# andrew-sha/CUDAFluidSimulator

Measured on AMD Instinct MI355X. Metric: particle-steps/sec (first 41 of the 100 steps of -m time), higher is better.
Workload: dtype f32

## Files before the change

cudafluidsimulator_amd/csrc/sph_api.hip:

```cpp
#include "sph_c_api.h"
#include "sph_device.h"

#include <hsa/hsa.h>
#include <hsa/hsa_ext_amd.h>

#include <algorithm>
#include <chrono>
#include <cmath>
#include <cstdio>
#include <cstdlib>
#include <cstring>
#include <string>
#include <vector>

namespace {

thread_local std::string g_create_error;

constexpr int kEventRing = 64;
constexpr int kCounterWords = 16 + 256 * 16;
constexpr size_t kCursorBytes = (size_t)SL_POOL_SHARDS * SL_CURSOR_STRIDE * sizeof(unsigned long long);

struct PairEvent {
    hipEvent_t a = nullptr, b = nullptr;
// ... 10 lines not shown

}

struct sph_handle {
    SphSettings settings{};
    SphOptions opt{};
    DevParams P{};
    int n = 0, cap = 0, device = 0;
    hipStream_t compute = nullptr, copy = nullptr;
    float4 *pos4[2] = {nullptr, nullptr};
    float4 *vel4[2] = {nullptr, nullptr};
    int cur = 0;
    int sorted = -1;
    SortWorkspace ws{};
    int sortedKeyBuf = 0;
    int2 *cellRange = nullptr;
    int2 *cellTable[2] = {nullptr, nullptr};
    int cellCur = 0;
    bool gridAhead = false;
    int2 *clickTable = nullptr;
    bool clickValid = false;
    bool aheadEnabled = true;
    StepEvents *aheadEv = nullptr;
    float *devPos[2] = {nullptr, nullptr};
    float *hostPos = nullptr;
    bool hostPosIsInit = false;
    float4 *stage[2] = {nullptr, nullptr};
    hipEvent_t stageFree[2] = {nullptr, nullptr};
    bool mappedPos = false;
    hipGraphExec_t stepGraph[2][3] = {{nullptr, nullptr, nullptr}, {nullptr, nullptr, nullptr}};
    StepEvents graphEv[2];
    bool graphEvPending[2] = {false, false};
    bool useGraph = false, capturing = false;
    int graphKeyBuf = 0;
    int graphCellCur[2] = {0, 0};
    hipEvent_t computeDone[2] = {nullptr, nullptr}, copyDone[2] = {nullptr, nullptr};
    bool copyPending[2] = {false, false};
    bool sdmaOk = false, stepTimed = false;
    hsa_agent_t hsaGpu{}, hsaCpu{};
    hsa_signal_t rbSig[2]{};
    bool rbPending[2] = {false, false};
    int rbDeferredSlot = -1;
    uint32_t sdmaEngine = 0;
    double hsaTickSeconds = 0;
    bool cursorClean = false;
    long long stepIndex = 0;
    float4 *force4 = nullptr;
    unsigned long long *pairCounter = nullptr;
    unsigned long long *pairHost = nullptr;
    StepEvents ring[kEventRing];
    int ringHead = 0;
    StepEvents *curEv = nullptr;
    SphKernelTimes kt{};
    float4 *pv8 = nullptr;
    uint32_t *maskPool = nullptr, *maskOff = nullptr;
    uint32_t *noneList = nullptr;
    uint32_t *hitCount = nullptr;
    int slabOwnedBegin = 0, slabOwnedEnd = 0;
    uint32_t *quiet = nullptr;
    float4 *quietVref = nullptr;
    unsigned long long *calm = nullptr;
    float4 *initPos4 = nullptr;
    SphOobLog *oobHost = nullptr;
    uint32_t oobSeen = 0;
    bool trace = false;
    double trEnqueue = 0, trSync = 0, trPost = 0, trBetween = 0, trPh[5] = {0, 0, 0, 0, 0};
    long long trSteps = 0;
    std::chrono::steady_clock::time_point trLastReturn{};
    hipEvent_t trBase = nullptr;
    int initZLayers = 0;
    bool useQuiet = true;
    uint64_t hitsRecorded = 0;
    unsigned long long *maskCursor = nullptr;
    unsigned long long maskCapacity = 0;
    bool external = false;
    hipStream_t ownCompute = nullptr;
    int *boundsDev = nullptr, *boundsHost = nullptr;
    int *partTiles = nullptr;
    PairEvent pairs[kPairRing];
    int pairHead = 0;
    int zLayers = 0;
    int tileChunkEnv = -1;
    int tileRotate = -1;
    RenderParams rp{};
    uint32_t *rDepth = nullptr, *rCount = nullptr, *rEdge = nullptr, *rRgb = nullptr;
    uint8_t *frameHost = nullptr;
    hipEvent_t frameDrawn = nullptr, frameCopied = nullptr;
    bool framePending = false;
    bool frameValid = false;
    double renderSeconds = 0;
    long long renderFrames = 0;
    bool ready = false;
    bool gridValid = false;
    int phase = 0;
    std::string err;
};

namespace {

#define HIPCHK(h, call)                                                               \
    do {                                                                              \
        hipError_t e__ = (call);                                                      \
        if (e__ != hipSuccess) {                                                      \
            (h)->err = std::string(#call) + ": " + hipGetErrorString(e__);            \
            return SPH_EHIP;                                                          \
        }                                                                             \
    } while (0)

#define SPH_ON_DEVICE(h)                                                              \
    do {                                                                              \
        int d__ = -1;                                                                 \
        if (hipGetDevice(&d__) != hipSuccess || d__ != (h)->device)                    \
            HIPCHK(h, hipSetDevice((h)->device));                                     \
    } while (0)

void report_oob(sph_handle *h) {
    if (!h || !h->oobHost) return;
    const uint32_t cnt = h->oobHost->count;
    if (cnt == h->oobSeen) return;
    const int D = h->P.D;
    const uint32_t shown = cnt < SPH_OOB_RECORDS ? cnt : SPH_OOB_RECORDS;
    for (uint32_t k = h->oobSeen < shown ? h->oobSeen : shown; k < shown; ++k) {
        const auto &r = h->oobHost->rec[k];
        const char axis[3] = {'x', 'y', 'z'};
        for (int a = 0; a < 3; ++a)
            if (r.cell[a] < 0 || r.cell[a] >= D)
                printf("OOB particle: %c = %d\n(%f, %f, %f)\n", axis[a], r.cell[a], r.pos[0], r.pos[1], r.pos[2]);
    }
    if (cnt > shown) printf("OOB particle: %u positions outside the grid so far (the first %u listed)\n", cnt, shown);
    fflush(stdout);
    h->oobSeen = cnt;
}

int fail(sph_handle *h, int code, const std::string &msg) {
    if (h) h->err = msg;
    else g_create_error = msg;
    return code;
}

float force_cut2(float h) {
    float h2 = h * h;
    float x = h2;
    for (int k = 0; k < 64; ++k) {
        float nx = std::nextafterf(x, INFINITY);
        if (sqrtf(nx) <= h) x = nx;
        else break;
    }
    return x;
}

void fill_params(sph_handle *h) {
    const SphSettings &s = h->settings;
    DevParams &P = h->P;
    P.h = s.h;
    P.h2 = s.h * s.h;
    P.vcoef = s.v_kernel_coeff;
    P.dcoef = s.d_kernel_coeff;
    P.boxDim = s.boxDim;
    P.boxHi = s.boxDim - s.h;
    P.dt = s.timestep;
    P.cut2 = force_cut2(s.h);
    P.D = (int)s.numCellsPerDim;
    P.morton = h->opt.key_order == SPH_KEY_MORTON ? 1 : 0;
    {
        SphSettings ref{};
        sph_default_settings(&ref, s.numParticles, s.randomInit);
// ... 401 lines not shown
    SPH_ON_DEVICE(h);
    if (h->external) return fail(h, SPH_ESTATE, "handle is in slab mode (external state)");
    if (n != h->n) return fail(h, SPH_EINVAL, "particle count differs from settings");
    const float hh = h->settings.h;
    const int D = h->P.D;
    std::vector<float4> p4((size_t)n), v4((size_t)n);
    int zmin = D, zmax = -1;
    for (int i = 0; i < n; ++i) {
        float x = pos[3 * i], y = pos[3 * i + 1], z = pos[3 * i + 2];
        const float qx = x / hh, qy = y / hh, qz = z / hh, Df = (float)D;
        if (!(qx >= 0.f && qx < Df && qy >= 0.f && qy < Df && qz >= 0.f && qz < Df && x >= 0.f && y >= 0.f && z >= 0.f))
            return fail(h, SPH_EINVAL, "position outside the simulation box");
        const int cz = (int)qz;
        zmin = cz < zmin ? cz : zmin;
        zmax = cz > zmax ? cz : zmax;
        uint32_t id = (uint32_t)i;
        float idbits;
        memcpy(&idbits, &id, 4);
        p4[i] = make_float4(x, y, z, idbits);
        v4[i] = vel ? make_float4(vel[3 * i], vel[3 * i + 1], vel[3 * i + 2], 0.f)
                    : make_float4(0.f, 0.f, 0.f, 0.f);
    }
    HIPCHK(h, hipStreamSynchronize(h->compute));
    HIPCHK(h, hipStreamSynchronize(h->copy));
    h->cur = 0;
    if (n > 0) {
        int rc = staged_upload(h, h->pos4[0], (size_t)n,
                               [&](size_t k, float4 *dst, size_t cnt) { memcpy(dst, p4.data() + k, cnt * sizeof(float4)); });
        if (!rc)
            rc = staged_upload(h, h->vel4[0], (size_t)n,
                               [&](size_t k, float4 *dst, size_t cnt) { memcpy(dst, v4.data() + k, cnt * sizeof(float4)); });
        if (rc) return rc;
    }
    HIPCHK(h, hipDeviceSynchronize());
    h->zLayers = zmax >= zmin ? zmax - zmin + 1 : 0;
    state_replaced(h);
    h->hostPosIsInit = false;
    if (h->hostPos && n > 0) memcpy(h->hostPos, pos, (size_t)n * 3 * sizeof(float));
    return SPH_OK;
}

static int slab_rotate(const sph_handle *h) { return h->tileRotate >= 0 ? h->tileRotate : 1; }

int tile_chunk(const sph_handle *h, int count, int layers) {
    if (h->tileChunkEnv >= 0) return h->tileChunkEnv;
    if (layers <= 0) return 0;
    const long long tiles = ((long long)count + 255) / 256;
    return (int)(tiles / (8ll * layers));
}

SweepArgs make_sweep_args(sph_handle *h) {
    SweepArgs A{};
    const int s = h->sorted;
    A.pos4 = h->pos4[s];
    A.vel4 = h->vel4[s];
    A.cellRange = h->cellRange;
    A.keys = h->ws.keys[h->sortedKeyBuf];
    A.pos_out = h->pos4[s ^ 1];
    A.vel_out = h->vel4[s ^ 1];
    A.host_order_pos = nullptr;
    A.force_out = h->force4;
    A.pairCounter = nullptr;
    A.i_begin = 0;
    A.i_end = h->n;
    A.i_origin = 0;
    A.i_begin2 = A.i_end2 = 0;
    A.nblk1 = 0;
    A.patchHalo = 0;
    A.n_all = h->n;
    A.tileChunk = tile_chunk(h, h->n, h->zLayers);
    A.tileRotate = h->tileRotate > 0 ? h->tileRotate : 0;
    A.maskPool = h->maskPool;
    A.maskOff = h->maskOff;
    A.noneList = h->noneList;
    A.hitCount = h->hitCount;
    A.maskCursor = h->maskCursor;
    A.maskCapacity = h->maskCapacity;
    A.pv8 = h->pv8;
    A.quiet = (h->useQuiet && h->quiet) ? h->quiet : nullptr;
    A.calm = h->calm;
    A.quietAll = A.quiet ? reinterpret_cast<uint32_t *>(h->quietVref + 1) : nullptr;
    A.quietHalo = nullptr;
    A.rhoToVel4 = h->external ? 1 : 0;
    A.listHead = reinterpret_cast<const int *>(h->cellRange);
    A.listNext = reinterpret_cast<const int *>(h->ws.vals[0]);
    return A;
}

GatherExtras gather_extras(sph_handle *h) {
    GatherExtras X;
    if (h->maskCursor) {
        X.cursor = h->maskCursor;
        X.cursorWords = (int)(kCursorBytes / sizeof(unsigned long long));
        h->cursorClean = true;
    }
    if (h->quiet && h->useQuiet) {
        X.vref = h->quietVref;
        X.calm = h->calm;
        X.quietAll = reinterpret_cast<uint32_t *>(h->quietVref + 1);
        if (h->external) {
            X.quietClear = h->quiet;
            X.quietWords = (int)(2 * (((size_t)h->cap + 63) / 64) + 2);
        }
    }
    return X;
}

int begin_step_events(sph_handle *h) {
    StepEvents &se = h->ring[h->ringHead];
    if (se.used) {
        int rc = resolve_events(h, se);
        if (rc) return rc;
    }
    se.used = true;
    se.counted = false;
    se.hasCopy = false;
    h->curEv = &se;
    h->ringHead = (h->ringHead + 1) % kEventRing;
    return SPH_OK;
}

int resolve_pair(sph_handle *h, PairEvent &pe) {
    if (!pe.used) return SPH_OK;
    float ms = 0.f;
    HIPCHK(h, hipEventSynchronize(pe.b));
    HIPCHK(h, hipEventElapsedTime(&ms, pe.a, pe.b));
    *pe.target += ms * 1e-3;
    pe.used = false;
    return SPH_OK;
}

int pair_begin(sph_handle *h, double *target, PairEvent **out, hipStream_t stream = nullptr) {
    PairEvent &pe = h->pairs[h->pairHead];
    int rc = resolve_pair(h, pe);
    if (rc) return rc;
    h->pairHead = (h->pairHead + 1) % kPairRing;
    pe.target = target;
    pe.used = true;
    HIPCHK(h, hipEventRecord(pe.a, stream ? stream : h->compute));
    *out = &pe;
    return SPH_OK;
}

int slab_range_ok(sph_handle *h, int buf, int i_begin, int i_end, int n_all) {
    if (!h->external || !h->pos4[0]) return fail(h, SPH_ESTATE, "sph_bind_buffers first");
    if ((buf != 0 && buf != 1) || i_begin < 0 || i_end < i_begin || n_all < i_end || n_all > h->cap)
        return fail(h, SPH_EINVAL, "bad slab range");
    return SPH_OK;
}

}

extern "C" {

int sph_set_stream(sph_handle *h, void *hip_stream) {
    if (!h) return SPH_EINVAL;
    SPH_ON_DEVICE(h);
    HIPCHK(h, hipStreamSynchronize(h->compute));
    if (!h->ownCompute) h->ownCompute = h->compute;
    h->compute = (hipStream_t)hip_stream;
    return SPH_OK;
}

int sph_bind_buffers(sph_handle *h, void *pos4_a, void *vel4_a, void *pos4_b, void *vel4_b,
                     int capacity) {
    if (!h) return SPH_EINVAL;
// ... 272 lines not shown
    float h = .1f;
    float h_pow_6 = (float)pow((double)h, 6.0);
    float h_pow_9 = (float)pow((double)h, 9.0);
    float v_kernel_coeff = 45.f / (3.14159265f * h_pow_6);
    float d_kernel_coeff = 315.f / (64.f * 3.14159265f * h_pow_9);
    memset(out, 0, sizeof(*out));
    out->randomInit = randomInit ? 1 : 0;
    out->numParticles = numParticles;
    out->h = h;
    out->v_kernel_coeff = v_kernel_coeff;
    out->d_kernel_coeff = d_kernel_coeff;
    out->boxDim = 10.f;
    out->numCellsPerDim = 100;
    out->timestep = (float).01;
    return SPH_OK;
}

int sph_initial_positions(const SphSettings *settings, float *pos_xyz) {
    if (!settings || (!pos_xyz && settings->numParticles > 0) || settings->numParticles < 0)
        return SPH_EINVAL;
    int written = init_positions_reference(*settings, pos_xyz);
    if (written < settings->numParticles) {
        fprintf(stderr,
                "sph: -i grid holds at most %d lattice points in the reference "
                "(simulator.cu:439-452); n=%d uses the dense-lattice EXTENSION\n",
                written, settings->numParticles);
        init_positions_dense(*settings, pos_xyz);
    }
    return SPH_OK;
}

int sph_create(const SphSettings *settings, const SphOptions *options, sph_handle **out) {
    if (!settings || !out) return fail(nullptr, SPH_EINVAL, "null argument");
    *out = nullptr;
    if (settings->numParticles < 0) return fail(nullptr, SPH_EINVAL, "numParticles < 0");
    if (!(settings->h > 0.f) || !(settings->numCellsPerDim >= 1.f) ||
        settings->numCellsPerDim > 1024.f)
        return fail(nullptr, SPH_EINVAL, "bad h / numCellsPerDim");
    int count = 0;
    if (hipGetDeviceCount(&count) != hipSuccess || count <= 0)
        return fail(nullptr, SPH_ENODEV,
                    "no HIP device: libsph_hip has no CPU fallback by design");
    sph_handle *h = new (std::nothrow) sph_handle();
    if (!h) return fail(nullptr, SPH_ENOMEM, "out of host memory");
    h->settings = *settings;
    if (options) {
        size_t sz = options->struct_size > 0 ? (size_t)options->struct_size : sizeof(SphOptions);
        memcpy(&h->opt, options, sz < sizeof(SphOptions) ? sz : sizeof(SphOptions));
    } else {
        h->opt.device = -1;
    }
    h->opt.struct_size = (int32_t)sizeof(SphOptions);
    if (h->opt.math_mode != SPH_MATH_STRICT && h->opt.math_mode != SPH_MATH_FAST) {
        delete h;
        return fail(nullptr, SPH_EINVAL, "unknown math_mode");
    }
    if (h->opt.sweep < SPH_SWEEP_LIST || h->opt.sweep > SPH_SWEEP_LINKED) {
        delete h;
        return fail(nullptr, SPH_EINVAL, "unknown sweep variant");
    }
    if (h->opt.math_mode == SPH_MATH_FAST &&
        (h->opt.sweep == SPH_SWEEP_DIRECT || h->opt.sweep == SPH_SWEEP_LINKED)) {
        delete h;
        return fail(nullptr, SPH_EINVAL, "SPH_MATH_FAST does not exist for SPH_SWEEP_DIRECT/LINKED");
    }
    if (h->opt.key_order != SPH_KEY_FLATTENED && h->opt.key_order != SPH_KEY_MORTON) {
        delete h;
        return fail(nullptr, SPH_EINVAL, "unknown key_order");
    }
    if (h->opt.key_order == SPH_KEY_MORTON &&
        (h->opt.sweep != SPH_SWEEP_DIRECT || (h->opt.flags & SPH_FLAG_EXTERNAL_STATE))) {
        delete h;
        return fail(nullptr, SPH_EINVAL, "SPH_KEY_MORTON is served by SPH_SWEEP_DIRECT, single domain, only");
    }
    if (h->opt.sweep == SPH_SWEEP_LINKED && (h->opt.flags & SPH_FLAG_EXTERNAL_STATE)) {
        delete h;
        return fail(nullptr, SPH_EINVAL, "SPH_SWEEP_LINKED is single-domain only");
    }
    h->n = settings->numParticles;
    if ((h->opt.flags & SPH_FLAG_EXTERNAL_STATE) && h->opt.capacity > 0) h->cap = h->opt.capacity;
    else h->cap = h->opt.capacity > h->n ? h->opt.capacity : h->n;
    if (const char *e = getenv("SPH_TILE_CHUNK")) h->tileChunkEnv = atoi(e);
    if (const char *e = getenv("SPH_XCD_ROTATE")) h->tileRotate = atoi(e);
    if (const char *e = getenv("SPH_STEP_TRACE")) h->trace = atoi(e) != 0;
    fill_params(h);
    int rc = SPH_OK;
    do {
        if (h->opt.device >= 0) {
            if (h->opt.device >= count) { rc = fail(nullptr, SPH_EINVAL, "device ordinal out of range"); break; }
            if (hipSetDevice(h->opt.device) != hipSuccess) { rc = fail(nullptr, SPH_EHIP, "hipSetDevice failed"); break; }
        }
        if (hipGetDevice(&h->device) != hipSuccess) { rc = fail(nullptr, SPH_EHIP, "hipGetDevice failed"); break; }
        if (hipStreamCreateWithFlags(&h->compute, hipStreamNonBlocking) != hipSuccess ||
            hipStreamCreateWithFlags(&h->copy, hipStreamNonBlocking) != hipSuccess) {
            rc = fail(nullptr, SPH_EHIP, "hipStreamCreate failed");
            break;
        }
        rc = alloc_device(h);
        if (rc) g_create_error = h->err;
    } while (0);
    if (rc) {
        sph_destroy(h);
        return rc;
    }
    *out = h;
    return SPH_OK;
}

void sph_destroy(sph_handle *h) {
    if (!h) return;
    if (h->trace && h->trSteps > 0)
        fprintf(stderr, "sph step trace (host, us per timed step over %lld steps): enqueue %.1f | wait for the compute stream %.1f | "
                        "after the wait %.1f | caller between two steps %.1f\n", h->trSteps, h->trEnqueue / h->trSteps * 1e6,
                h->trSync / h->trSteps * 1e6, h->trPost / h->trSteps * 1e6, h->trBetween / (h->trSteps > 1 ? h->trSteps - 1 : 1) * 1e6),
        fprintf(stderr, "  enqueue split: events %.1f | grid %.1f | density %.1f | force %.1f | read-back %.1f\n", h->trPh[0] / h->trSteps * 1e6,
                h->trPh[1] / h->trSteps * 1e6, h->trPh[2] / h->trSteps * 1e6, h->trPh[3] / h->trSteps * 1e6, h->trPh[4] / h->trSteps * 1e6);
    if (h->compute) (void)hipStreamSynchronize(h->compute);
    if (h->copy) (void)hipStreamSynchronize(h->copy);
    if (h->hsaTickSeconds > 0) {
        (void)sdma_wait(h, 0);
        (void)sdma_wait(h, 1);
        (void)hsa_signal_destroy(h->rbSig[0]);
        (void)hsa_signal_destroy(h->rbSig[1]);
        (void)hsa_shut_down();
    }
    for (int b = 0; b < 2; ++b) {
        if (h->pos4[b] && !h->external) (void)hipFree(h->pos4[b]);
        if (h->vel4[b] && !h->external) (void)hipFree(h->vel4[b]);
        if (h->ws.keys[b]) (void)hipFree(h->ws.keys[b]);
        if (h->ws.vals[b]) (void)hipFree(h->ws.vals[b]);
        if (h->devPos[b] && !h->mappedPos) (void)hipFree(h->devPos[b]);
        if (h->computeDone[b]) (void)hipEventDestroy(h->computeDone[b]);
        if (h->copyDone[b]) (void)hipEventDestroy(h->copyDone[b]);
    }
    if (h->ws.blockHist) (void)hipFree(h->ws.blockHist);
    if (h->ws.digitTotal) (void)hipFree(h->ws.digitTotal);
    for (auto &t : h->cellTable) if (t) (void)hipFree(t);
    if (h->hostPos) (void)hipHostFree(h->hostPos);
    for (int b = 0; b < 2; ++b) {
        if (h->stage[b]) (void)hipHostFree(h->stage[b]);
        if (h->stageFree[b]) (void)hipEventDestroy(h->stageFree[b]);
    }
    if (h->force4) (void)hipFree(h->force4);
    if (h->pairCounter) (void)hipFree(h->pairCounter);
    if (h->pairHost) (void)hipHostFree(h->pairHost);
    for (auto &se : h->ring) {
        for (auto &e : se.e) if (e) (void)hipEventDestroy(e);
        for (auto &e : se.c) if (e) (void)hipEventDestroy(e);
    }
    for (auto &se : h->graphEv) {
        for (auto &e : se.e) if (e) (void)hipEventDestroy(e);
        for (auto &e : se.c) if (e) (void)hipEventDestroy(e);
    }
    for (auto &gs : h->stepGraph)
        for (auto &g : gs)
            if (g) (void)hipGraphExecDestroy(g);
    if (h->pv8) (void)hipFree(h->pv8);
    if (h->maskPool) (void)hipFree(h->maskPool);
    if (h->maskOff) (void)hipFree(h->maskOff);
    if (h->noneList) (void)hipFree(h->noneList);
    if (h->hitCount) (void)hipFree(h->hitCount);
    if (h->maskCursor) (void)hipFree(h->maskCursor);
    if (h->quiet) (void)hipFree(h->quiet);
    if (h->quietVref) (void)hipFree(h->quietVref);
    if (h->calm) (void)hipFree(h->calm);
    if (h->initPos4) (void)hipFree(h->initPos4);
// ... 822 lines not shown
```

cudafluidsimulator_amd/csrc/sph_device.h:

```cpp
#pragma once

#include <hip/hip_runtime.h>
#include <stdint.h>

#define SPH_WAVE 64

#define SPH_MASS 0.02f
#define SPH_GAS_CONSTANT 1.f
#define SPH_REST_DENSITY 1000.f
#define SPH_VISCOSITY 1.f
#define SPH_GRAVITY -9.8f
#define SPH_ELASTICITY 0.5f
#define SPH_EPS_F (1e-4f)
#define SPH_PUSH_STRENGTH (5.f)
#define SPH_BOX_MAX_X (600)
#define SPH_BOX_MIN_X (200)
#define SPH_BOX_MAX_Y (450)
#define SPH_BOX_MIN_Y (150)

struct DevParams {
    float h;
    float h2;
    float vcoef;
    float dcoef;
// ... 38 lines not shown
    const float4 *velSample;
    float4 *vrefOut;
};
size_t sph_sort_workspace_blocks(int n);
int sph_sort_pairs(const SortWorkspace &ws, int n, int bits, hipStream_t s);
struct DevParams;
int sph_sort_cells(const SortWorkspace &ws, const DevParams &P, const float4 *pos4, int n, int bits,
                   hipStream_t s, int2 *cellRange, int numCells);

void sph_launch_hash(const DevParams &P, const float4 *pos4, uint32_t *keys,
                     uint32_t *vals, int n, hipStream_t s);
struct Thresholds { uint32_t v[8]; };
struct GatherExtras {
    unsigned long long *cursor = nullptr;
    int cursorWords = 0;
    int *bounds = nullptr;
    const float4 *vref = nullptr;
    unsigned long long *calm = nullptr;
    uint32_t *quietAll = nullptr;
    uint32_t *quietClear = nullptr;
    int quietWords = 0;
    Thresholds thr{};
    int nthr = 0;
};
void sph_launch_gather(const float4 *pos_in, const float4 *vel_in,
                       const uint32_t *perm, const uint32_t *sorted_keys,
                       float4 *pos_out, float4 *vel_out, float4 *pv8, int2 *cellRange, int n,
                       hipStream_t s, const GatherExtras &X = GatherExtras());
void sph_launch_lower_bounds(const uint32_t *sorted_keys, int n, Thresholds thr, int nthr,
                             int *bounds_dev, hipStream_t s);
void sph_launch_classify(const DevParams &P, const float4 *pos4, Thresholds thr, int nthr,
                         uint32_t *keys, uint32_t *vals, int n, hipStream_t s);
void sph_launch_partition(const DevParams &P, const float4 *pos_in, const float4 *vel_in, float4 *pos_out,
                          float4 *vel_out, Thresholds thr, int nthr, int n, int *tileCount, int *bounds_dev,
                          hipStream_t s);
size_t sph_partition_tiles(int n);
void sph_launch_gather_plain(const float4 *pos_in, const float4 *vel_in, const uint32_t *perm,
                             float4 *pos_out, float4 *vel_out, int n, hipStream_t s);
struct SegmentTable {
    const float4 *spos[8];
    const float4 *svel[8];
    int dst[8];
    int prefix[9];
    int n;
};
void sph_launch_copy_segments(const SegmentTable &T, float4 *dpos, float4 *dvel, hipStream_t s);
void sph_launch_click(const DevParams &P, const int2 *cellRange, float4 *vel4,
                      int mx, int my, hipStream_t s, int zlo = 0, int zhi = 1 << 30);

#define SL_POOL_SHARDS 64
#define SL_CURSOR_STRIDE 32

struct SweepArgs {
    const float4 *pos4;
    float4 *vel4;
    const int2 *cellRange;
    const uint32_t *keys;
    float4 *pos_out;
    float4 *vel_out;
    float *host_order_pos;
    float4 *force_out;
    unsigned long long *pairCounter;
    unsigned long long *stampCounter;
    int i_begin, i_end;
    int i_origin;
    int i_begin2, i_end2;
    int nblk1;
    int n_all;
    int patchHalo;
    int tileChunk;
    int tileRotate;
    uint32_t *maskPool;
    uint32_t *maskOff;
    uint32_t *hitCount;
    unsigned long long *maskCursor;
    uint32_t *noneList;
    unsigned long long maskCapacity;
    float4 *pv8;
    uint32_t *quiet;
    const unsigned long long *calm;
    uint32_t *quietAll;
    const uint32_t *quietHalo;
    int rhoToVel4;
    const int *listHead;
    const int *listNext;
};
void sph_launch_halo_quiet(const float4 *pv8, int lo_end, int hi_begin, int n_all, const float4 *vref,
                           const uint32_t *ownedQuiet, uint32_t *haloQuiet, hipStream_t s);
void sph_launch_link_build(const DevParams &P, const float4 *pos4, int *head, int *next, int n,
                           hipStream_t s);
void sph_launch_density_linked(const DevParams &P, const SweepArgs &A, hipStream_t s);
void sph_launch_force_linked(const DevParams &P, const SweepArgs &A, hipStream_t s);
void sph_launch_density_list(const DevParams &P, const SweepArgs &A, int mathMode, hipStream_t s);
void sph_launch_force_list(const DevParams &P, const SweepArgs &A, int mathMode, hipStream_t s);
void sph_launch_patch_halo(const SweepArgs &A, hipStream_t s);
void sph_launch_density(const DevParams &P, const SweepArgs &A, int mathMode,
                        int sweep, hipStream_t s);
void sph_launch_force(const DevParams &P, const SweepArgs &A, int mathMode,
                      int sweep, hipStream_t s);

struct RenderParams {
    int width, height;
    float Wf, Hf;
    int radius;
    int shade;
};
void sph_launch_render_edges(const RenderParams &R, uint32_t *edge, hipStream_t s);
void sph_launch_render(const RenderParams &R, const float4 *pos4, int n, bool plain, uint32_t *depth, uint32_t *count,
                       const uint32_t *edge, uint32_t *rgb, hipStream_t s);
```

cudafluidsimulator_amd/csrc/sweeps_list.hip:

```cpp
#include "sweep_common.h"

#define SL_NONE 0xFFFFFFFFu

#ifndef SL_WINDOW
#define SL_WINDOW 160
#endif
#ifndef SL_K1_THREADS
#define SL_K1_THREADS 64
#endif

#ifndef SL_K1_WAVES
#define SL_K1_WAVES 6
#endif
__device__ __forceinline__ void sl_store_quiet(const SweepArgs &A, int i, bool valid, float rho, int lane) {
    const unsigned long long calm = A.calm[(i - lane) >> 6];
    const float prs = fmaxf(0.f, SPH_GAS_CONSTANT * (rho - SPH_REST_DENSITY));
    const bool q = valid && prs == 0.f && ((calm >> lane) & 1ull);
    const unsigned long long qb = __ballot(q), vb = __ballot(valid);
    if (lane == 0) {
        reinterpret_cast<unsigned long long *>(A.quiet)[(i - lane) >> 6] = qb;
        if (A.quietAll && qb != vb) *A.quietAll = 0u;
    }
}
__device__ __forceinline__ uint32_t sl_quiet_window(const uint32_t *__restrict__ quiet, uint32_t j) {
// ... 131 lines not shown
                const int jsr = R.jsr, len = R.len;
                const float4 *cur = stage + (jsr - R.u0);
                const float4 *gcur = A.pos4 + jsr;
                uint32_t m = 0;
                int k = 0;
                auto trip = [&](const float4 (&pj)[SW_UNROLL]) {
#pragma unroll
                    for (int u = 0; u < SW_UNROLL; ++u) {
                        float dx = pi.x - pj[u].x;
                        float dy = pi.y - pj[u].y;
                        float dz = pi.z - pj[u].z;
                        float dist2;
                        float draw;
                        if (FAST) {
                            dist2 = __builtin_fmaf(dz, dz, __builtin_fmaf(dy, dy, dx * dx));
                            draw = h2v - dist2;
                            const float diff = fmaxf(draw, 0.f);
                            rho = __builtin_fmaf((massv * dcv) * (diff * diff), diff, rho);
                        } else {
                            dist2 = dx * dx + dy * dy + dz * dz;
                            draw = h2v - dist2;
                            float diff;
                            asm("v_max_f32_e32 %0, 0, %1" : "=v"(diff) : "v"(draw));
                            rho += massv * (dcv * diff * diff * diff);
                        }
                        if (SAMECUT) {
                            m = __builtin_amdgcn_alignbit(m, __float_as_uint(draw), 31);
                            continue;
                        }
                        asm("v_cmp_ngt_f32_e32 vcc, %1, %2\n\tv_addc_co_u32_e32 %0, vcc, %0, %0, vcc"
                            : "+v"(m)
                            : "v"(dist2), "v"(cut2r)
                            : "vcc");
                    }
#pragma unroll
                    for (int u = 0; u < SW_UNROLL; ++u) asm volatile("" ::"v"(pj[u].w));
                    if (((k + SW_UNROLL) & 31) == 0) {
                        if (SAMECUT) emit((uint32_t)(jsr + (k & ~31)), ~__builtin_bitreverse32(m));
                        else emit((uint32_t)(jsr + (k & ~31)), __builtin_bitreverse32(m));
                        m = 0;
                    }
                };
                if (R.staged) {
                    for (; __ballot(k < len); k += SW_UNROLL) {
                        float4 pj[SW_UNROLL];
#pragma unroll
                        for (int u = 0; u < SW_UNROLL; ++u) {
                            const float4 *p = (k + u < len) ? cur + k : sent;
                            pj[u] = p[u];
                        }
                        trip(pj);
                    }
                } else {
                    for (; __ballot(k < len); k += SW_UNROLL) {
                        float4 pj[SW_UNROLL];
#pragma unroll
                        for (int u = 0; u < SW_UNROLL; ++u) {
                            const bool in = k + u < len;
                            pj[u] = gcur[in ? k + u : 0];
                            pj[u].x = in ? pj[u].x : 1e18f;
                        }
                        trip(pj);
                    }
                }
                if ((k & 31) != 0) {
                    if (SAMECUT) emit((uint32_t)(jsr + (k & ~31)), (~__builtin_bitreverse32(m)) >> (32 - (k & 31)));
                    else emit((uint32_t)(jsr + (k & ~31)), __builtin_bitreverse32(m) >> (32 - (k & 31)));
                }
                __builtin_amdgcn_fence(__ATOMIC_ACQUIRE, "wavefront");
                __builtin_amdgcn_wave_barrier();
            }
        }
    }
    if (ok && valid) {
        if (pending) myq[(size_t)qidx * SPH_WAVE] = make_uint4(pj0, pm0, 0u, 0u);
        else if (qidx < Q) myq[(size_t)qidx * SPH_WAVE] = make_uint4(0u, 0u, 0u, 0u);
    }
    if (valid) {
        rho = fmaxf(rho, SPH_EPS_F);
        if (A.rhoToVel4) A.vel4[i].w = rho;
        A.pv8[2 * (size_t)i + 1].w = rho;
    }
    if (A.quiet) sl_store_quiet(A, i, valid, rho, lane);
    if (A.hitCount && valid) A.hitCount[i] = hcount;
}

#ifndef SL_SORT_SHIFT
#define SL_SORT_SHIFT 3
#endif
#define SL_DEAL_THREADS 256
#define SL_DEAL_ROWS SL_DEAL_THREADS
#define SL_DEAL_WINDOW (SL_DEAL_ROWS + SL_WINDOW - SPH_WAVE)
static_assert(SL_WINDOW >= SPH_WAVE, "the dealt sweep needs the window");

template <bool FAST, bool SLIM>
__global__ __launch_bounds__(SL_DEAL_THREADS) void k_force_dealt(DevParams P, SweepArgs A) {
    __shared__ uint32_t sortBase[128];
    __shared__ uint16_t rowOf[SL_DEAL_ROWS];
    __shared__ float4 win[2 * SL_DEAL_WINDOW];
    const int t = threadIdx.x, lane = t & 63;
    const bool second = (int)blockIdx.x >= A.nblk1;
    const int rb = second ? A.i_begin2 : A.i_begin, re = second ? A.i_end2 : A.i_end;
    const int chunk = A.tileChunk > 0 ? max(A.tileChunk * 256 / SL_DEAL_ROWS, 1) : 0;
    const int group = ((rb - A.i_origin) >> 6) / (SL_DEAL_ROWS / SPH_WAVE) +
                      xcd_tile(second ? (int)blockIdx.x - A.nblk1 : (int)blockIdx.x,
                               second ? (int)gridDim.x - A.nblk1 : A.nblk1, chunk, A.tileRotate);
    const int R0 = A.i_origin + group * SL_DEAL_ROWS;
    const unsigned long long *const quiet64 = reinterpret_cast<const unsigned long long *>(A.quiet);

    unsigned long long qw = 0ull;
    bool inPlace = false;
    if (A.quiet) {
        const int r0 = R0 + (t & ~63);
        const int lo = max(rb - r0, 0), hi = min(re - r0, 64);
        const unsigned long long vm = hi > lo ? ((hi - lo == 64 ? ~0ull : (1ull << (hi - lo)) - 1ull) << lo) : 0ull;
        if (vm) qw = quiet64[r0 >> 6];
        inPlace = __syncthreads_and((qw & vm) == vm) != 0;
    }
    if (!inPlace) {
        for (int b = t; b < 128; b += SL_DEAL_THREADS) sortBase[b] = 0u;
        __syncthreads();
        const int row = R0 + t;
        const bool counted = row >= rb && row < re && !((qw >> lane) & 1ull);
        const uint32_t bucket = min((counted ? A.hitCount[row] : 0u) >> SL_SORT_SHIFT, 127u);
        const uint32_t slot = atomicAdd(&sortBase[bucket], 1u);
        __syncthreads();
        if (t < SPH_WAVE) {
            const uint32_t a = sortBase[2 * t], b = sortBase[2 * t + 1];
            uint32_t incl = a + b;
#pragma unroll
            for (int off = 1; off < SPH_WAVE; off <<= 1) {
                const uint32_t up = __shfl_up(incl, off);
                incl += t >= off ? up : 0u;
            }
            const uint32_t excl = incl - (a + b);
            sortBase[2 * t] = excl;
            sortBase[2 * t + 1] = excl + a;
        }
        __syncthreads();
        rowOf[sortBase[bucket] + slot] = (uint16_t)t;
    }

    const bool allQuiet = A.quietAll && __builtin_amdgcn_readfirstlane(*A.quietAll) != 0u &&
                          (!A.quietHalo || __builtin_amdgcn_readfirstlane(*A.quietHalo) != 0u);
    const int w0 = max(R0 - (SL_WINDOW - SPH_WAVE) / 2, 0);
    int wlen = max(min(SL_DEAL_WINDOW, A.n_all - w0), 0);
    {
        bool wanted = !allQuiet && wlen > 0;
        if (wanted && A.quiet) {
            const int k0 = w0 >> 6, k1 = (w0 + wlen - 1) >> 6;
            wanted = k0 + t <= k1 && quiet64[k0 + t] != ~0ull;
        }
        if (__syncthreads_or(wanted)) {
            for (int k = t; k < 2 * wlen; k += SL_DEAL_THREADS) win[k] = A.pv8[2 * (size_t)w0 + k];
            __syncthreads();
        } else {
            wlen = 0;
        }
    }

    {
        const int i = R0 + (inPlace ? t : (int)rowOf[t]);
        const bool inRange = i >= rb && i < re;
        const int iSafe = inRange ? i : rb;
        float4 pi = A.pv8[2 * (size_t)iSafe];
        const float4 vi = A.pv8[2 * (size_t)iSafe + 1];
// ... 62 lines not shown
    }
#define SD_USE(j, p, v)                                                        \
    if ((unsigned)((j)-w0) < (unsigned)wlen) {                                 \
        p = win[2 * ((j)-w0)];                                                 \
        v = win[2 * ((j)-w0) + 1];                                             \
    }                                                                          \
    body(p, v);
                float4 p0 = make_float4(0, 0, 0, 0), v0 = p0, p1 = p0, v1 = p0;
                int j0 = pop();
                SD_FETCH(j0, p0, v0)
                int j1 = pop();
                SD_FETCH(j1, p1, v1)
                for (;;) {
                    SD_USE(j0, p0, v0)
                    if (!__ballot(live)) { SD_USE(j1, p1, v1) break; }
                    j0 = pop();
                    SD_FETCH(j0, p0, v0)
                    SD_USE(j1, p1, v1)
                    if (!__ballot(live)) { SD_USE(j0, p0, v0) break; }
                    j1 = pop();
                    SD_FETCH(j1, p1, v1)
                }
#undef SD_FETCH
#undef SD_USE
#undef SD_UNDEF4
            }
        }
        if (valid) {
            float vx = vi.x, vy = vi.y, vz = vi.z;
            integrate_particle(P, pi, vx, vy, vz, F, vi.w);
            store_particle(A, i, pi, vx, vy, vz, vi.w, F);
        }
    }
}

__global__ __launch_bounds__(256) void k_halo_quiet(const float4 *__restrict__ pv8, int lo_end, int hi_begin, int n_all,
                                                    const float4 *__restrict__ vref, const uint32_t *__restrict__ ownedQuiet,
                                                    uint32_t *__restrict__ haloQuiet) {
    if (*ownedQuiet == 0u) return;
    const int t = blockIdx.x * blockDim.x + threadIdx.x;
    if (t >= lo_end + (n_all - hi_begin)) return;
    const int j = t < lo_end ? t : hi_begin + (t - lo_end);
    const float4 v = pv8[2 * (size_t)j + 1], r = *vref;
    const float prs = fmaxf(0.f, SPH_GAS_CONSTANT * (v.w - SPH_REST_DENSITY));
    if (!(prs == 0.f && v.x == r.x && v.y == r.y && v.z == r.z)) *haloQuiet = 0u;
}
void sph_launch_halo_quiet(const float4 *pv8, int lo_end, int hi_begin, int n_all, const float4 *vref,
                           const uint32_t *ownedQuiet, uint32_t *haloQuiet, hipStream_t s) {
    const int rows = lo_end + (n_all - hi_begin);
    if (rows > 0) k_halo_quiet<<<(rows + 255) / 256, 256, 0, s>>>(pv8, lo_end, hi_begin, n_all, vref, ownedQuiet, haloQuiet);
}

__global__ __launch_bounds__(256) void k_count_hits(SweepArgs A) {
    const int i = A.i_begin + blockIdx.x * blockDim.x + threadIdx.x;
    uint32_t n = 0, dropped = 0;
    if (i < A.i_end) {
        const int wv = (i - A.i_origin) >> 6;
        const uint32_t baseq = A.maskOff[2 * (size_t)wv];
        const int Q = (int)A.maskOff[2 * (size_t)wv + 1];
        if (baseq != SL_NONE) {
            const uint4 *q4 = reinterpret_cast<const uint4 *>(A.maskPool) + baseq + (threadIdx.x & 63);
            const bool qi = A.quiet && ((A.quiet[i >> 5] >> (i & 31)) & 1u);
            for (int q = 0; q < Q; ++q) {
                const uint4 t = q4[(size_t)q * SPH_WAVE];
                n += (uint32_t)__builtin_popcount(t.y) + (uint32_t)__builtin_popcount(t.w);
                if (qi)
                    dropped += (uint32_t)__builtin_popcount(t.y & sl_quiet_window(A.quiet, t.x)) +
                               (uint32_t)__builtin_popcount(t.w & sl_quiet_window(A.quiet, t.z));
                if (t.w == 0u) break;
            }
        }
    }
    n = wave_sum_u32(n);
    dropped = wave_sum_u32(dropped);
    if ((threadIdx.x & 63) == 0 && n) {
        atomicAdd(A.pairCounter + 16 + (blockIdx.x & 255) * 16 + 15, (unsigned long long)n);
        atomicAdd(A.pairCounter + 16 + (blockIdx.x & 255) * 16 + 14, (unsigned long long)(n - dropped));
    }
}

void sph_launch_density_list(const DevParams &P, const SweepArgs &A, int mathMode, hipStream_t s) {
    int cnt = A.i_end - A.i_begin;
    if (cnt <= 0) return;
    int blocks = (A.i_end - A.i_origin + SL_K1_THREADS - 1) / SL_K1_THREADS;
    const bool same = P.cut2 == P.h2;
    if (mathMode == 1) {
        if (same) k_density_mask_lds<true, true><<<blocks, SL_K1_THREADS, 0, s>>>(P, A);
        else k_density_mask_lds<true, false><<<blocks, SL_K1_THREADS, 0, s>>>(P, A);
    } else {
        if (same) k_density_mask_lds<false, true><<<blocks, SL_K1_THREADS, 0, s>>>(P, A);
        else k_density_mask_lds<false, false><<<blocks, SL_K1_THREADS, 0, s>>>(P, A);
    }
    if (A.pairCounter) k_count_hits<<<(cnt + 255) / 256, 256, 0, s>>>(A);
}

#define SL_FALLBACK_BLOCKS 512
template <bool FAST, bool SLIM>
__global__ __launch_bounds__(SPH_WAVE) void k_force_fallback(DevParams P, SweepArgs A) {
    const unsigned count = (unsigned)A.maskCursor[1];
    for (unsigned idx = blockIdx.x; idx < count; idx += gridDim.x) {
    const int i = A.i_origin + (int)A.noneList[idx] * SPH_WAVE + (int)threadIdx.x;
    const bool mine = (i >= A.i_begin && i < A.i_end) || (i >= A.i_begin2 && i < A.i_end2);
    if (!__ballot(mine)) continue;
    const int iSafe = mine ? i : A.i_begin;
    float4 pi = A.pv8[2 * (size_t)iSafe];
    const float4 vi = A.pv8[2 * (size_t)iSafe + 1];
    const float prs_i = fmaxf(0.f, SPH_GAS_CONSTANT * (vi.w - SPH_REST_DENSITY));
    int3 c = sweep_cell(P, pi.x, pi.y, pi.z);
    int js[9], je[9];
    load_runs(P, A.cellRange, c, mine, js, je);
    ForceAcc F = {0.f, 0.f, 0.f};
#pragma unroll
    for (int r = 0; r < 9; ++r)
        for (int j = js[r]; j < je[r]; ++j) {
            if (FAST) force_pair_fast(P, pi.x, pi.y, pi.z, vi.x, vi.y, vi.z, prs_i, A.pv8[2 * (size_t)j], A.pv8[2 * (size_t)j + 1], F);
            else force_pair<SLIM>(P, pi.x, pi.y, pi.z, vi.x, vi.y, vi.z, prs_i, A.pv8[2 * (size_t)j], A.pv8[2 * (size_t)j + 1], F);
        }
    if (mine) {
        float vx = vi.x, vy = vi.y, vz = vi.z;
        integrate_particle(P, pi, vx, vy, vz, F, vi.w);
        store_particle(A, i, pi, vx, vy, vz, vi.w, F);
    }
    }
}

__global__ void k_patch_pv8(const float4 *__restrict__ vel4, float4 *__restrict__ pv8, int i_begin,
                            int i_end, int n_all) {
    int t = blockIdx.x * blockDim.x + threadIdx.x;
    int j = t < i_begin ? t : i_end + (t - i_begin);
    if (j < n_all) pv8[2 * (size_t)j + 1] = vel4[j];
}

void sph_launch_patch_halo(const SweepArgs &A, hipStream_t s) {
    const int halo = A.i_begin + (A.n_all - A.i_end);
    if (halo > 0) k_patch_pv8<<<(halo + 255) / 256, 256, 0, s>>>(A.vel4, A.pv8, A.i_begin, A.i_end, A.n_all);
}

void sph_launch_force_list(const DevParams &P, const SweepArgs &A, int mathMode, hipStream_t s) {
    SweepArgs B = A;
    if (B.i_end2 <= B.i_begin2) B.i_begin2 = B.i_end2 = 0;
    if (B.i_end <= B.i_begin) {
        B.i_begin = B.i_begin2;
        B.i_end = B.i_end2;
        B.i_begin2 = B.i_end2 = 0;
    }
    if (B.i_end <= B.i_begin) return;
    if (B.patchHalo) sph_launch_patch_halo(B, s);
    const int wpb = SL_DEAL_ROWS / SPH_WAVE, threads = SL_DEAL_THREADS;
    auto blocks_of = [&](int a, int b) {
        if (b <= a) return 0;
        const int w0 = (a - B.i_origin) >> 6, w1 = (b - B.i_origin + 63) >> 6;
        return (w1 + wpb - 1) / wpb - w0 / wpb;
    };
    B.nblk1 = blocks_of(B.i_begin, B.i_end);
    const int fblocks = B.nblk1 + blocks_of(B.i_begin2, B.i_end2);
    const int blocks = SL_FALLBACK_BLOCKS;
    if (mathMode == 1) {
        k_force_dealt<true, true><<<fblocks, threads, 0, s>>>(P, B);
        k_force_fallback<true, true><<<blocks, SPH_WAVE, 0, s>>>(P, B);
    } else if (P.slimDiv) {
        k_force_dealt<false, true><<<fblocks, threads, 0, s>>>(P, B);
        k_force_fallback<false, true><<<blocks, SPH_WAVE, 0, s>>>(P, B);
    } else {
        k_force_dealt<false, false><<<fblocks, threads, 0, s>>>(P, B);
        k_force_fallback<false, false><<<blocks, SPH_WAVE, 0, s>>>(P, B);
    }
}
```

Measured before the change: 4.531 billion.

## Stage neighbor positions per workgroup in LDS for the density mask sweep

```diff
diff --git a/cudafluidsimulator_amd/csrc/sph_api.hip b/cudafluidsimulator_amd/csrc/sph_api.hip
--- a/cudafluidsimulator_amd/csrc/sph_api.hip
+++ b/cudafluidsimulator_amd/csrc/sph_api.hip
@@ -116,6 +116,7 @@
     int zLayers = 0;
     int tileChunkEnv = -1;
     int tileRotate = -1;
+    int densityPerWave = 0;
     RenderParams rp{};
     uint32_t *rDepth = nullptr, *rCount = nullptr, *rEdge = nullptr, *rRgb = nullptr;
     uint8_t *frameHost = nullptr;
@@ -683,6 +684,7 @@
     A.quietAll = A.quiet ? reinterpret_cast<uint32_t *>(h->quietVref + 1) : nullptr;
     A.quietHalo = nullptr;
     A.rhoToVel4 = h->external ? 1 : 0;
+    A.densityPerWave = h->densityPerWave;
     A.listHead = reinterpret_cast<const int *>(h->cellRange);
     A.listNext = reinterpret_cast<const int *>(h->ws.vals[0]);
     return A;
@@ -1121,6 +1123,7 @@
     else h->cap = h->opt.capacity > h->n ? h->opt.capacity : h->n;
     if (const char *e = getenv("SPH_TILE_CHUNK")) h->tileChunkEnv = atoi(e);
     if (const char *e = getenv("SPH_XCD_ROTATE")) h->tileRotate = atoi(e);
+    if (const char *e = getenv("SPH_DENSITY_PER_WAVE")) h->densityPerWave = atoi(e) != 0;
     if (const char *e = getenv("SPH_STEP_TRACE")) h->trace = atoi(e) != 0;
     fill_params(h);
     int rc = SPH_OK;
diff --git a/cudafluidsimulator_amd/csrc/sph_device.h b/cudafluidsimulator_amd/csrc/sph_device.h
--- a/cudafluidsimulator_amd/csrc/sph_device.h
+++ b/cudafluidsimulator_amd/csrc/sph_device.h
@@ -144,6 +144,7 @@
     uint32_t *quietAll;
     const uint32_t *quietHalo;
     int rhoToVel4;
+    int densityPerWave;
     const int *listHead;
     const int *listNext;
 };
diff --git a/cudafluidsimulator_amd/csrc/sweeps_list.hip b/cudafluidsimulator_amd/csrc/sweeps_list.hip
--- a/cudafluidsimulator_amd/csrc/sweeps_list.hip
+++ b/cudafluidsimulator_amd/csrc/sweeps_list.hip
@@ -237,6 +237,198 @@
         A.pv8[2 * (size_t)i + 1].w = rho;
     }
     if (A.quiet) sl_store_quiet(A, i, valid, rho, lane);
+    if (A.hitCount && valid) A.hitCount[i] = hcount;
+}
+
+#ifndef SL_WG_CAP
+#define SL_WG_CAP 1024
+#endif
+#define SL_WG_THREADS 256
+#define SL_WG_WAVES (SL_WG_THREADS / SPH_WAVE)
+#define SL_WG_DONE 0x7fffffff
+static_assert(SL_WG_CAP % 32 == 0 && SL_WG_CAP >= 64, "a piece holds whole words and always lets its first lane advance");
+
+__device__ __forceinline__ int wave_min_i32(int v) {
+#pragma unroll
+    for (int off = 32; off > 0; off >>= 1) v = min(v, __shfl_xor(v, off));
+    return v;
+}
+
+template <bool FAST, bool SAMECUT>
+__global__ __launch_bounds__(SL_WG_THREADS, SL_K1_WAVES)
+void k_density_mask_wg(DevParams P, SweepArgs A) {
+    __shared__ float4 stage[SL_WG_CAP + SW_UNROLL];
+    __shared__ int2 vote[2][SL_WG_WAVES];
+    const int lane = threadIdx.x & 63, w = threadIdx.x >> 6;
+    const int wv = xcd_tile(blockIdx.x, gridDim.x, A.tileChunk, A.tileRotate) * SL_WG_WAVES + w;
+    const int i = A.i_origin + wv * SPH_WAVE + lane;
+    const bool valid = i >= A.i_begin && i < A.i_end;
+    const bool anyValid = __ballot(valid) != 0ull;
+    float4 pi = valid ? A.pos4[i] : make_float4(0, 0, 0, 0);
+    int3 c = sweep_cell(P, pi.x, pi.y, pi.z);
+    int js[9], je[9];
+    load_runs(P, A.cellRange, c, valid, js, je);
+
+    int words = 0;
+    uint32_t pairs = 0;
+#pragma unroll
+    for (int r = 0; r < 9; ++r) {
+        words += (je[r] - js[r] + 31) >> 5;
+        pairs += (uint32_t)(je[r] - js[r]);
+    }
+    const int Q = __builtin_amdgcn_readfirstlane((wave_max_i32(words) + 1) >> 1);
+    const int shard = wv & (SL_POOL_SHARDS - 1);
+    unsigned long long base = 0;
+    if (lane == 0 && anyValid) base = atomicAdd(A.maskCursor + shard * SL_CURSOR_STRIDE, (unsigned long long)Q * SPH_WAVE);
+    base = (unsigned long long)__builtin_amdgcn_readfirstlane((unsigned)(base >> 32)) << 32 |
+           (unsigned long long)__builtin_amdgcn_readfirstlane((unsigned)base);
+    const unsigned long long subCap = A.maskCapacity / SL_POOL_SHARDS;
+    const bool ok = base + (unsigned long long)Q * SPH_WAVE <= subCap;
+    base += (unsigned long long)shard * subCap;
+    if (lane == 0 && anyValid) {
+        A.maskOff[2 * (size_t)wv] = ok ? (uint32_t)base : SL_NONE;
+        A.maskOff[2 * (size_t)wv + 1] = (uint32_t)Q;
+        if (!ok) A.noneList[atomicAdd(A.maskCursor + 1, 1ull)] = (uint32_t)wv;
+    }
+    uint4 *const myq = reinterpret_cast<uint4 *>(A.maskPool) + (ok ? base : 0ull) + lane;
+    if (A.pairCounter) {
+        uint32_t s = wave_sum_u32(pairs);
+        if (lane == 0) atomicAdd(A.pairCounter + 16 + (wv & 255) * 16, (unsigned long long)s);
+    }
+
+    if (threadIdx.x < SW_UNROLL) stage[SL_WG_CAP + threadIdx.x] = make_float4(1e18f, 1e18f, 1e18f, 0.f);
+    const float4 *const sent = stage + SL_WG_CAP;
+    float rho = 0.f;
+    float h2v = P.h2, dcv = P.dcoef, cut2r = P.cut2, massv = SPH_MASS;
+    asm volatile("" : "+v"(h2v), "+v"(dcv), "+v"(cut2r), "+v"(massv));
+    uint32_t pj0 = 0, pm0 = 0;
+    bool pending = false;
+    int qidx = 0;
+    uint32_t hcount = 0;
+    auto emit = [&](uint32_t jbase, uint32_t mask) {
+        if (ok && mask != 0) {
+            hcount += (uint32_t)__builtin_popcount(mask);
+            if (!pending) {
+                pj0 = jbase;
+                pm0 = mask;
+                pending = true;
+            } else {
+                myq[(size_t)qidx * SPH_WAVE] = make_uint4(pj0, pm0, jbase, mask);
+                ++qidx;
+                pending = false;
+            }
+        }
+    };
+    int round = 0;
+#pragma unroll 1
+    for (int r = 0; r < 9; ++r) {
+        int js0 = js[0], jer = je[0];
+#pragma unroll
+        for (int q = 1; q < 9; ++q) {
+            js0 = (r == q) ? js[q] : js0;
+            jer = (r == q) ? je[q] : jer;
+        }
+        const bool nonempty = valid && jer > js0;
+        const int total = nonempty ? jer - js0 : 0;
+        int done = 0;
+        const unsigned long long mm = __ballot(nonempty);
+        int first = SL_WG_DONE, uend = 0;
+        if (mm) {
+            first = __builtin_amdgcn_readlane(js0, __ffsll((long long)mm) - 1);
+            uend = __builtin_amdgcn_readlane(jer, 63 - __clzll((long long)mm));
+        }
+        for (;;) {
+            if (lane == 0) vote[round][w] = make_int2(first, uend);
+            __syncthreads();
+            int p0 = SL_WG_DONE, pe = 0;
+#pragma unroll
+            for (int q = 0; q < SL_WG_WAVES; ++q) {
+                const int2 v = vote[round][q];
+                p0 = min(p0, v.x);
+                pe = max(pe, v.y);
+            }
+            p0 = __builtin_amdgcn_readfirstlane(p0);
+            pe = __builtin_amdgcn_readfirstlane(pe);
+            round ^= 1;
+            if (p0 == SL_WG_DONE) break;
+            const int plen = min(SL_WG_CAP, pe - p0);
+            for (int k = threadIdx.x; k < plen; k += SL_WG_THREADS) stage[k] = A.pos4[p0 + k];
+            __syncthreads();
+            {
+                const int at = js0 + done;
+                const bool rem = done < total && at < p0 + plen;
+                const int room = p0 + plen - at;
+                const int len = !rem ? 0 : (total - done <= room ? total - done : (room & ~31));
+                const int jsr = rem ? at : p0;
+                done += len;
+                const float4 *cur = stage + (jsr - p0);
+                uint32_t m = 0;
+                int k = 0;
+                auto trip = [&](const float4 (&pj)[SW_UNROLL]) {
+#pragma unroll
+                    for (int u = 0; u < SW_UNROLL; ++u) {
+                        float dx = pi.x - pj[u].x;
+                        float dy = pi.y - pj[u].y;
+                        float dz = pi.z - pj[u].z;
+                        float dist2;
+                        float draw;
+                        if (FAST) {
+                            dist2 = __builtin_fmaf(dz, dz, __builtin_fmaf(dy, dy, dx * dx));
+                            draw = h2v - dist2;
+                            const float diff = fmaxf(draw, 0.f);
+                            rho = __builtin_fmaf((massv * dcv) * (diff * diff), diff, rho);
+                        } else {
+                            dist2 = dx * dx + dy * dy + dz * dz;
+                            draw = h2v - dist2;
+                            float diff;
+                            asm("v_max_f32_e32 %0, 0, %1" : "=v"(diff) : "v"(draw));
+                            rho += massv * (dcv * diff * diff * diff);
+                        }
+                        if (SAMECUT) {
+                            m = __builtin_amdgcn_alignbit(m, __float_as_uint(draw), 31);
+                            continue;
+                        }
+                        asm("v_cmp_ngt_f32_e32 vcc, %1, %2\n\tv_addc_co_u32_e32 %0, vcc, %0, %0, vcc"
+                            : "+v"(m)
+                            : "v"(dist2), "v"(cut2r)
+                            : "vcc");
+                    }
+#pragma unroll
+                    for (int u = 0; u < SW_UNROLL; ++u) asm volatile("" ::"v"(pj[u].w));
+                    if (((k + SW_UNROLL) & 31) == 0) {
+                        if (SAMECUT) emit((uint32_t)(jsr + (k & ~31)), ~__builtin_bitreverse32(m));
+                        else emit((uint32_t)(jsr + (k & ~31)), __builtin_bitreverse32(m));
+                        m = 0;
+                    }
+                };
+                for (; __ballot(k < len); k += SW_UNROLL) {
+                    float4 pj[SW_UNROLL];
+#pragma unroll
+                    for (int u = 0; u < SW_UNROLL; ++u) {
+                        const float4 *p = (k + u < len) ? cur + k : sent;
+                        pj[u] = p[u];
+                    }
+                    trip(pj);
+                }
+                if ((k & 31) != 0) {
+                    if (SAMECUT) emit((uint32_t)(jsr + (k & ~31)), (~__builtin_bitreverse32(m)) >> (32 - (k & 31)));
+                    else emit((uint32_t)(jsr + (k & ~31)), __builtin_bitreverse32(m) >> (32 - (k & 31)));
+                }
+            }
+            if (pe - p0 <= SL_WG_CAP) break;
+            first = __builtin_amdgcn_readfirstlane(wave_min_i32(done < total ? js0 + done : SL_WG_DONE));
+        }
+    }
+    if (ok && valid) {
+        if (pending) myq[(size_t)qidx * SPH_WAVE] = make_uint4(pj0, pm0, 0u, 0u);
+        else if (qidx < Q) myq[(size_t)qidx * SPH_WAVE] = make_uint4(0u, 0u, 0u, 0u);
+    }
+    if (valid) {
+        rho = fmaxf(rho, SPH_EPS_F);
+        if (A.rhoToVel4) A.vel4[i].w = rho;
+        A.pv8[2 * (size_t)i + 1].w = rho;
+    }
+    if (A.quiet && anyValid) sl_store_quiet(A, i, valid, rho, lane);
     if (A.hitCount && valid) A.hitCount[i] = hcount;
 }
 
@@ -465,8 +657,20 @@
 void sph_launch_density_list(const DevParams &P, const SweepArgs &A, int mathMode, hipStream_t s) {
     int cnt = A.i_end - A.i_begin;
     if (cnt <= 0) return;
+    const bool same = P.cut2 == P.h2;
+    if (A.densityPerWave == 0) {
+        const int wg = (A.i_end - A.i_origin + SL_WG_THREADS - 1) / SL_WG_THREADS;
+        if (mathMode == 1) {
+            if (same) k_density_mask_wg<true, true><<<wg, SL_WG_THREADS, 0, s>>>(P, A);
+            else k_density_mask_wg<true, false><<<wg, SL_WG_THREADS, 0, s>>>(P, A);
+        } else {
+            if (same) k_density_mask_wg<false, true><<<wg, SL_WG_THREADS, 0, s>>>(P, A);
+            else k_density_mask_wg<false, false><<<wg, SL_WG_THREADS, 0, s>>>(P, A);
+        }
+        if (A.pairCounter) k_count_hits<<<(cnt + 255) / 256, 256, 0, s>>>(A);
+        return;
+    }
     int blocks = (A.i_end - A.i_origin + SL_K1_THREADS - 1) / SL_K1_THREADS;
-    const bool same = P.cut2 == P.h2;
     if (mathMode == 1) {
         if (same) k_density_mask_lds<true, true><<<blocks, SL_K1_THREADS, 0, s>>>(P, A);
         else k_density_mask_lds<true, false><<<blocks, SL_K1_THREADS, 0, s>>>(P, A);
```

Result: no change. 4.519 billion (-0.3%).
